# srv/pcl_feature_extraction

Hardware: AMD Instinct MI355X
Metric: Mpoints/s through NARF keypoint + FPFH descriptor on 1M-pt cloud (higher is better)
Workload: dtype f32; 1 GPU; configs[2] 1M-pt synthetic room, NARF(support 0.2) + normals(r 0.05) + FPFH(r 0.08) at the keypoints; image=640x480, parallelism=scan-per-gpu x1, descriptor_rows=83

## Files before the change

pcl_feature_extraction_amd/csrc/pfx_grid.hip:

```cpp
#include <algorithm>
#include <cstdlib>
#include <cstring>
#include <rocprim/rocprim.hpp>

#include "pfx_internal.h"

namespace pfx {
namespace {

__device__ __forceinline__ uint32_t f2ord(float f) {
  uint32_t u = __float_as_uint(f);
  return (u & 0x80000000u) ? ~u : (u | 0x80000000u);
}
__host__ __device__ __forceinline__ float ord2f(uint32_t u) {
  uint32_t b = (u & 0x80000000u) ? (u & 0x7fffffffu) : ~u;
  float f;
  memcpy(&f, &b, 4);
  return f;
}

constexpr int kBboxBlocks = 1024;
__global__ void __launch_bounds__(256) k_bbox(const float* __restrict__ x, const float* __restrict__ y,
                                              const float* __restrict__ z, int64_t n,
                                              uint32_t* __restrict__ mm) {
// ... 257 lines not shown

}

static bool bbox_dev(pfx_ctx* ctx, Grid& g, const float* d_x, const float* d_y, const float* d_z, int64_t n,
                     double lo[3], double hi[3]) {
  hipStream_t st = ctx->stream;
  uint32_t* mm = g.b_minmax.as<uint32_t>(6 * (kBboxBlocks + 1));
  const int blocks = (int)std::min<int64_t>(std::max<int64_t>(ceil_div(n, 1024), 1), kBboxBlocks);
  {
    TimeScope ts(ctx, "grid_bbox");
    k_bbox<<<blocks, 256, 0, st>>>(d_x, d_y, d_z, n, mm);
    k_bbox_reduce<<<1, 256, 0, st>>>(mm, blocks);
    check_launch("k_bbox");
  }
  uint32_t* h = ctx->readback<uint32_t>();
  PFX_HIP(hipMemcpyAsync(h, mm + 6 * blocks, sizeof(uint32_t) * 6, hipMemcpyDeviceToHost, st));
  ctx->sync_spin(st);
  uint32_t r[6];
  for (int d = 0; d < 6; ++d) r[d] = h[d];
  const bool any = r[0] != 0xffffffffu && r[3] != 0u;
  for (int d = 0; d < 3; ++d) {
    lo[d] = any ? ord2f(r[d]) : 0.0;
    hi[d] = any ? ord2f(r[3 + d]) : 0.0;
  }
  return any;
}

void points_bbox(pfx_ctx* ctx, Grid& g, const float* d_x, const float* d_y, const float* d_z, int64_t n,
                 double lo[3], double hi[3]) {
  bbox_dev(ctx, g, d_x, d_y, d_z, n, lo, hi);
}

void build_grid(pfx_ctx* ctx, Grid& g, const float* d_x, const float* d_y, const float* d_z,
                int64_t n, double radius, bool use_hint) {
  PFX_CHECK(n >= 0 && n < (int64_t(1) << 31), "point count must be in [0, 2^31)");
  PFX_CHECK(radius > 0.0, "radius must be > 0");
  if (&g == &ctx->grid_b) {
    ctx->prep_x = nullptr;
    ctx->prep_n = -1;
    ctx->prep_qx = nullptr;
    ctx->prep_nq = -1;
  }
  hipStream_t st = ctx->stream;
  ++g.gen;
  g.n = n;
  g.ux = d_x; g.uy = d_y; g.uz = d_z;
  double lo[3] = {0, 0, 0}, hi[3] = {0, 0, 0};
  g.oob = nullptr;
  g.hint_user |= use_hint;
  if (use_hint && g.have_hint && n > 0) {
    for (int d = 0; d < 3; ++d) {
      lo[d] = g.hint_lo[d];
      hi[d] = g.hint_hi[d];
    }
    g.oob = g.b_oob.as<int>(1);
  } else if (n > 0) {
    bbox_dev(ctx, g, d_x, d_y, d_z, n, lo, hi);
    for (int d = 0; d < 3; ++d) {
      const double m = 0.1 * (hi[d] - lo[d]) + 2.0 * radius;
      g.hint_lo[d] = lo[d] - m;
      g.hint_hi[d] = hi[d] + m;
    }
    g.have_hint = true;
  }
  double cell = radius * (1.0 + 1e-6);
  const double max_cells = double(1 << 26);
  int64_t dims[3];
  for (int it = 0; it < 64; ++it) {
    for (int d = 0; d < 3; ++d) dims[d] = (int64_t)std::floor((hi[d] - lo[d]) / cell) + 1;
// ... 50 lines not shown
    check_launch("k_count_keys");
    PFX_HIP(rocprim::exclusive_scan(tmp, scan_bytes, g.cell_start, g.cell_start, int32_t(0), (size_t)m,
                                    rocprim::plus<int32_t>(), st));
    k_count_scatter<<<(unsigned)blocks, kCountBlock, 0, st>>>(d_x, d_y, d_z, n, (uint32_t)C, keys, vals, g.cell_start,
                                                              scr, keys2);
    k_count_order<<<(unsigned)ceil_div(n, 256), 256, 0, st>>>(scr, keys2, n, (uint32_t)C, g.cell_start, g.perm, g.sx,
                                                              g.sy, g.sz, g.sp, g.oob);
    check_launch("k_count_order");
    return;
  }

  using SortCfg = rocprim::radix_sort_config<rocprim::default_config, rocprim::default_config,
                                             rocprim::default_config, 0>;
  int bits = 1;
  while ((int64_t(1) << bits) <= C) ++bits;
  size_t sort_bytes = 0, scan_bytes = 0;
  PFX_HIP(rocprim::radix_sort_pairs<SortCfg>(nullptr, sort_bytes, (uint32_t*)nullptr, (uint32_t*)nullptr,
                                    (uint32_t*)nullptr, (uint32_t*)nullptr, (size_t)std::max<int64_t>(n, 1),
                                    0, bits, st));
  auto rev = rocprim::make_reverse_iterator(static_cast<int32_t*>(nullptr));
  PFX_HIP(rocprim::inclusive_scan(nullptr, scan_bytes, rev, rev, (size_t)(C + 1), rocprim::minimum<int32_t>(), st));
  void* tmp = g.b_tmp.get(std::max(sort_bytes, scan_bytes) + 16);
  g.cell_start = g.b_start.as<int32_t>(C + 2);
  {
    TimeScope ts(ctx, "grid_build");
    k_fill_i32<<<(unsigned)std::min<int64_t>(ceil_div(C + 2, 256), 2048), 256, 0, st>>>(g.cell_start, C + 2,
                                                                                       (int32_t)n);
    if (g.oob) k_fill_i32<<<1, 64, 0, st>>>(g.oob, 1, 0);
    if (n > 0) {
      k_cell_keys<<<(unsigned)ceil_div(n, 256), 256, 0, st>>>(d_x, d_y, d_z, n, cm, keys, vals, g.oob);
      check_launch("k_cell_keys");
      PFX_HIP(rocprim::radix_sort_pairs<SortCfg>(tmp, sort_bytes, keys, keys2, vals,
                                        reinterpret_cast<uint32_t*>(g.perm), (size_t)n, 0, bits, st));
      k_mark_starts<<<(unsigned)ceil_div(n, 256), 256, 0, st>>>(keys2, n, g.cell_start);
      auto r = rocprim::make_reverse_iterator(g.cell_start + C + 1);
      PFX_HIP(rocprim::inclusive_scan(tmp, scan_bytes, r, r, (size_t)(C + 1), rocprim::minimum<int32_t>(), st));
      k_gather_sorted<<<(unsigned)ceil_div(n, 256), 256, 0, st>>>(
          d_x, d_y, d_z, n, reinterpret_cast<uint32_t*>(g.perm), g.sx, g.sy, g.sz, g.sp);
      check_launch("k_gather_sorted");
    }
  }
  if (!g.oob && n > 0 && g.hint_user) {
    int* d_fat = g.b_fat.as<int>(1);
    if (!g.h_fat) PFX_HIP(hipHostMalloc((void**)&g.h_fat, 64, hipHostMallocDefault));
    if (!g.fat_ev) PFX_HIP(hipEventCreateWithFlags(&g.fat_ev, hipEventDisableTiming));
    if (g.fat_pending) PFX_HIP(hipEventSynchronize(g.fat_ev));
    k_fill_i32<<<1, 64, 0, st>>>(d_fat, 1, 0);
    k_fat_cells<<<(unsigned)ceil_div(C, 256), 256, 0, st>>>(g.cell_start, C, d_fat);
    check_launch("k_fat_cells");
    PFX_HIP(hipMemcpyAsync(g.h_fat, d_fat, sizeof(int), hipMemcpyDeviceToHost, st));
    PFX_HIP(hipEventRecord(g.fat_ev, st));
    g.fat_pending = true;
  }
}

}
```

pcl_feature_extraction_amd/csrc/pfx_internal.h:

```cpp
#pragma once
#include <hip/hip_runtime.h>
#include <stdint.h>
#include <cstdlib>

#include <map>
#include <stdexcept>
#include <string>
#include <vector>

#include "../../include/pfx.h"

namespace pfx {

struct Error : std::runtime_error {
  pfx_status code;
  Error(pfx_status c, const std::string& m) : std::runtime_error(m), code(c) {}
};

#define PFX_HIP(expr)                                                                   \
  do {                                                                                  \
    hipError_t _e = (expr);                                                             \
    if (_e != hipSuccess)                                                               \
      throw ::pfx::Error(PFX_ERR_DEVICE, std::string(#expr) + ": " + hipGetErrorString(_e)); \
  } while (0)
// ... 129 lines not shown
  pfx::FpfhReadback* fpfh_rb() {
    if (!fpfh_rb_mem) PFX_HIP(hipHostMalloc(&fpfh_rb_mem, sizeof(pfx::FpfhReadback), hipHostMallocDefault));
    return static_cast<pfx::FpfhReadback*>(fpfh_rb_mem);
  }
  void* pfh_rb_mem = nullptr;
  bool pfh_pending = false;
  void* spin_rb_mem = nullptr;
  bool spin_pending = false;
  void* rift_rb_mem = nullptr;
  bool igrad_pending = false, rift_pending = false;
  void* sc_rb_mem = nullptr;
  bool sc_pending = false, lrf_pending = false;
  void* moments_rb_mem = nullptr;
  bool moments_pending = false, pcurv_pending = false;
  int64_t sc_rnd_n = 0;
  hipStream_t side = nullptr;
  hipEvent_t fork_ev[2] = {nullptr, nullptr};
  hipEvent_t spin_ev = nullptr;
  void sync_spin(hipStream_t st) {
    if (!spin_ev) PFX_HIP(hipEventCreateWithFlags(&spin_ev, hipEventDisableTiming));
    PFX_HIP(hipEventRecord(spin_ev, st));
    hipError_t e;
    while ((e = hipEventQuery(spin_ev)) == hipErrorNotReady) {
    }
    PFX_HIP(e);
  }
  void ensure_side() {
    if (side) return;
    int prio = 0;
    if (stream) PFX_HIP(hipStreamGetPriority(stream, &prio));
    PFX_HIP(hipStreamCreateWithPriority(&side, hipStreamNonBlocking, prio));
    for (auto& e : fork_ev) PFX_HIP(hipEventCreateWithFlags(&e, hipEventDisableTiming));
  }
  void* host_rb = nullptr;
  template <class T> T* readback() {
    if (!host_rb) PFX_HIP(hipHostMalloc(&host_rb, 4096, hipHostMallocDefault));
    return static_cast<T*>(host_rb);
  }
  void* host_scratch = nullptr;
  size_t host_scratch_bytes = 0;
  void* pinned(size_t need) {
    if (need > host_scratch_bytes) {
      if (host_scratch) {
        PFX_HIP(hipStreamSynchronize(stream));
        PFX_HIP(hipHostFree(host_scratch));
      }
      host_scratch_bytes = need + need / 2 + 4096;
      PFX_HIP(hipHostMalloc(&host_scratch, host_scratch_bytes, hipHostMallocDefault));
    }
    return host_scratch;
  }
};

namespace pfx {

struct TimeScope {
  pfx_ctx* ctx;
  hipEvent_t a = nullptr, b = nullptr;
  std::string name;
  TimeScope(pfx_ctx* c, std::string n, bool stage = false) : ctx(c), name(std::move(n)) {
    if (ctx->timer.enabled && (stage || !ctx->timer.stages_only)) {
      a = ctx->timer.take();
      b = ctx->timer.take();
      PFX_HIP(hipEventRecord(a, ctx->stream));
    }
  }
  ~TimeScope() {
    if (a) {
      (void)hipEventRecord(b, ctx->stream);
      ctx->timer.pending.push_back(KernelTimer::Pending{a, b, name});
    }
  }
};

inline void check_launch(const char* what) {
  hipError_t e = hipGetLastError();
  if (e != hipSuccess)
    throw Error(PFX_ERR_DEVICE, std::string("launch ") + what + ": " + hipGetErrorString(e));
}

inline int64_t ceil_div(int64_t a, int64_t b) { return (a + b - 1) / b; }

void build_grid(pfx_ctx* ctx, Grid& g, const float* d_x, const float* d_y, const float* d_z,
                int64_t n, double radius, bool use_hint = false);
void points_bbox(pfx_ctx* ctx, Grid& g, const float* d_x, const float* d_y, const float* d_z, int64_t n,
                 double lo[3], double hi[3]);
inline void note_grid_word(pfx_ctx* ctx, const Grid& g, int word) {
  if (!(word & kGridFatBit)) return;
  g.fat = true;
  ++ctx->stats["grid_fat_fallbacks"];
}
inline GridView view(const Grid& g) {
  GridView v;
  v.sx = g.sx; v.sy = g.sy; v.sz = g.sz; v.sp = g.sp; v.perm = g.perm; v.cell_start = g.cell_start;
  v.ux = g.ux; v.uy = g.uy; v.uz = g.uz;
  v.inv = g.dinv; v.ox = g.dox; v.oy = g.doy; v.oz = g.doz; v.nx = g.nx; v.ny = g.ny; v.nz = g.nz;
  return v;
}

void normals_dev(pfx_ctx* ctx, const float* x, const float* y, const float* z, int64_t n,
                 double r, const float vp[3], float* nx, float* ny, float* nz, float* curv);
void normals_lists_dev(pfx_ctx* ctx, const float* x, const float* y, const float* z, int64_t n, double r,
                       float* nx, float* ny, float* nz, float* curv);
void normals_chains_dev(pfx_ctx* ctx, pfx_ctx* owner, const uint8_t* mask, int want, const float vp[3], float* nx,
                        float* ny, float* nz, float* curv);
void normals_release(pfx_ctx* ctx);
void normals_grid_launch_dev(pfx_ctx* ctx, const float* x, const float* y, const float* z, int64_t n, double r);
void normals_launch_dev(pfx_ctx* ctx, const float* x, const float* y, const float* z, int64_t n, double r,
                        const float vp[3], float* nx, float* ny, float* nz, float* curv);
bool normals_finish_dev(pfx_ctx* ctx);
void normals_prepare_dev(pfx_ctx* ctx, const float* x, const float* y, const float* z, int64_t n, double r);
void normals_subset_dev(pfx_ctx* ctx, const float* x, const float* y, const float* z, int64_t n, double r,
                        const uint8_t* mask, int want, const float vp[3], float* nx, float* ny, float* nz,
                        float* curv);
void normals_fast_dev(pfx_ctx* ctx, const float* x, const float* y, const float* z, int64_t n, double r,
                      const float vp[3], float* nx, float* ny, float* nz, float* curv);
double cloud_resolution_dev(pfx_ctx* ctx, const float* x, const float* y, const float* z, int64_t n);
// ... 99 lines not shown
```

pcl_feature_extraction_amd/csrc/pfx_nblist.h:

```cpp
#pragma once
#include "pfx_internal.h"

namespace pfx {

constexpr uint32_t kEntryOffMask = 0x0fffffffu;
__host__ __device__ __forceinline__ int entry_run(uint32_t e) { return (int)(e >> 28); }
__host__ __device__ __forceinline__ uint32_t entry_off(uint32_t e) { return e & kEntryOffMask; }
constexpr uint8_t kLgCompact = 0x80;

__host__ __device__ __forceinline__ uint32_t widen_entry16(uint32_t e16) {
  return ((e16 >> 12) << 28) | (e16 & 0xfffu);
}
constexpr int kLaneMaxCompact = 2048;
__device__ __forceinline__ uint32_t list_entry(const uint32_t* list, int64_t off, int lgr, int m) {
  const int64_t i = off + ((int64_t)m << (lgr & 0x7f));
  return (lgr & kLgCompact) ? widen_entry16(reinterpret_cast<const uint16_t*>(list)[i]) : list[i];
}

struct NbLists {
  int64_t nq = 0;
  int64_t total = 0;
  int64_t long_total = 0;
  int64_t long_nq = 0;
  int64_t slots = 0;
  const int32_t* qpos = nullptr;
  const int64_t* off = nullptr;
  const int32_t* cnt = nullptr;
  const uint8_t* lg = nullptr;
  const uint32_t* list = nullptr;
  bool compact = false;
  int64_t list_cap = 0;
  const uint32_t* skeys = nullptr;
  const int64_t* nq_dev = nullptr;
};

__device__ __forceinline__ int64_t nq_of(const NbLists& L) { return L.nq_dev ? *L.nq_dev : L.nq; }

constexpr int kLongList = 1024;

struct NormalsState {
  NbLists L;
  int64_t n = 0;
  const float *x = nullptr, *y = nullptr, *z = nullptr;
  double r = 0.0;
  bool ready = false;
  uint64_t grid_gen = 0;
  bool pending = false;
  uint64_t grid_ahead_gen = 0;
  const float *grid_ahead_x = nullptr, *grid_ahead_y = nullptr, *grid_ahead_z = nullptr;
  int64_t grid_ahead_n = 0;
  double grid_ahead_r = 0.0;
  float vp[3] = {0.f, 0.f, 0.f};
  float *nx = nullptr, *ny = nullptr, *nz = nullptr, *curv = nullptr;
};

void build_lists(pfx_ctx* ctx, const Grid& g, const uint8_t* mask, double radius, bool sorted, NbLists& out,
                 const char* tag, bool defer = false, int want = 1, bool compact = false, bool gate = false);
bool build_lists_check(pfx_ctx* ctx, const Grid& g, NbLists& out, const char* tag);

}
```

pcl_feature_extraction_amd/csrc/pfx_nblist.hip:

```cpp
#include <cstdlib>
#include <cstring>
#include <rocprim/rocprim.hpp>

#include "pfx_nblist.h"
#include "pfx_neighbors.h"

namespace pfx {
namespace {

constexpr int kQ = 16;
typedef float pf2 __attribute__((ext_vector_type(2)));
constexpr int kArena = 16384;
constexpr int kArenaQuery = 16384;
constexpr int kTcapSmall = 384, kTcapSparse = 1280, kTcapDense = 8000;
constexpr int kCapQuery = 4096, kBucketsQuery = 1024;
constexpr int kCapMid8 = 8192, kBucketsMid8 = 1024;
constexpr int kCapMid = 16384, kBucketsMid = 2048;
#ifndef PFX_HUGE_BLOCKS
#define PFX_HUGE_BLOCKS 1024
#endif
constexpr int kCapHuge = 1 << 18, kBucketsHuge = 4096, kHugeBlocks = PFX_HUGE_BLOCKS;
#ifndef PFX_NT_QUERY
#define PFX_NT_QUERY 512
#endif
// ... 155 lines not shown
                                                    const int64_t* __restrict__ ntiles_ptr,
                                                    int32_t* __restrict__ recs, int64_t n,
                                                    int32_t* __restrict__ wide, int* __restrict__ counts) {
  const int64_t t = blockIdx.x * (int64_t)blockDim.x + threadIdx.x;
  const int64_t ntiles = *ntiles_ptr;
  const int lane = threadIdx.x & 63;
  int cls = -1, qn = 0;
  int32_t start = 0;
  Runs R;
  if (t < ntiles) {
    start = tiles[t];
    const int64_t next = (t + 1 < ntiles) ? tiles[t + 1] : *nq_ptr;
    qn = (int)(next - start < kQ ? next - start : kQ);
    const int T = block_runs(g, skeys[qpos[start]], R);
    cls = T <= kTcapSmall ? 3 : (T <= kTcapSparse ? 0 : (T <= kTcapDense ? 1 : 2));
  }
#pragma unroll
  for (int c = 0; c < 4; ++c) {
    const uint64_t m = __ballot(cls == c);
    if (!m) continue;
    int base = 0;
    const int ci = c == 3 ? kTilesSmall : (c == 2 ? kTilesWide : (c == 1 ? kTilesDense : kTilesSparse));
    if (lane == __builtin_ctzll(m)) base = atomicAdd(&counts[ci], __popcll(m));
    base = __shfl(base, __builtin_ctzll(m));
    if (cls == c) {
      const int64_t slot = base + __popcll(m & lanemask_lt());
      const int64_t at = c == 3 ? slot : (c == 0 ? n + slot : (c == 1 ? 2 * n - 1 - slot : n - 1 - slot));
      rec_write(recs + at * kRecInts, R, start, qn);
      if (c == 2) wide[slot] = (int32_t)at;
    }
  }
}

constexpr int kCoopTiles = 16;
constexpr int kCellsPerThread = 8;
constexpr int64_t kCellsMinGrid = int64_t(256) * 256 * kCellsPerThread;
__device__ __forceinline__ int tile_class(int T) {
  return T <= kTcapSmall ? 3 : (T <= kTcapSparse ? 0 : (T <= kTcapDense ? 1 : 2));
}
__global__ void __launch_bounds__(256) k_tile_cells(GridView g, int64_t ncells, int32_t* __restrict__ recs, int64_t n,
                                                    int32_t* __restrict__ wide, int* __restrict__ counts) {
  __shared__ int s_wave[4][4];
  __shared__ int s_base[4];
  const int lane = threadIdx.x & 63, wv = threadIdx.x >> 6;
  const int64_t c0 = (blockIdx.x * (int64_t)blockDim.x + threadIdx.x) * kCellsPerThread;
  int32_t st[kCellsPerThread + 1];
#pragma unroll
  for (int j = 0; j <= kCellsPerThread; ++j) st[j] = g.cell_start[c0 + j <= ncells ? c0 + j : ncells];
  int cnt[4] = {0, 0, 0, 0};
  unsigned cls_bits = 0;
#pragma unroll
  for (int j = 0; j < kCellsPerThread; ++j) {
    const int m = st[j + 1] - st[j];
    if (m > 0) {
      Runs R;
      const int cls = tile_class(block_runs(g, (uint32_t)(c0 + j), R));
      cls_bits |= (unsigned)cls << (2 * j);
#pragma unroll
      for (int k = 0; k < 4; ++k) cnt[k] += cls == k ? (m + kQ - 1) / kQ : 0;
    }
  }
  int first[4];
#pragma unroll
  for (int k = 0; k < 4; ++k) {
    const int incl = wave_incl_scan(cnt[k]);
    first[k] = incl - cnt[k];
    if (lane == 63) s_wave[k][wv] = incl;
  }
  __syncthreads();
  if (threadIdx.x < 4) {
    const int k = threadIdx.x;
    const int total = s_wave[k][0] + s_wave[k][1] + s_wave[k][2] + s_wave[k][3];
    const int ci = k == 3 ? kTilesSmall : (k == 2 ? kTilesWide : (k == 1 ? kTilesDense : kTilesSparse));
    s_base[k] = total ? atomicAdd(&counts[ci], total) : 0;
  }
  __syncthreads();
#pragma unroll
  for (int k = 0; k < 4; ++k) {
    first[k] += s_base[k];
    for (int w = 0; w < wv; ++w) first[k] += s_wave[k][w];
  }
  auto emit = [&](const Runs& Rc, int k, int slot, int32_t q0, int qn) {
    const int64_t at = k == 3 ? slot : (k == 0 ? n + slot : (k == 1 ? 2 * n - 1 - slot : n - 1 - slot));
    rec_write(recs + at * kRecInts, Rc, q0, qn);
    if (k == 2) wide[slot] = (int32_t)at;
  };
#pragma unroll
  for (int j = 0; j < kCellsPerThread; ++j) {
    const int32_t s = st[j], m = st[j + 1] - st[j];
    const int nt = (m + kQ - 1) / kQ, cls = (int)((cls_bits >> (2 * j)) & 3u);
    Runs R;
#pragma unroll
    for (int r = 0; r < 9; ++r) R.start[r] = 0;
#pragma unroll
    for (int r = 0; r < 10; ++r) R.pref[r] = 0;
    int slot = 0;
    if (m > 0) {
      block_runs(g, (uint32_t)(c0 + j), R);
      slot = cls == 3 ? first[3] : (cls == 2 ? first[2] : (cls == 1 ? first[1] : first[0]));
#pragma unroll
      for (int k = 0; k < 4; ++k) first[k] += cls == k ? nt : 0;
      if (nt <= kCoopTiles)
        for (int i = 0; i < nt; ++i) emit(R, cls, slot + i, s + kQ * i, min(kQ, m - kQ * i));
    }
    uint64_t big = __ballot(m > 0 && nt > kCoopTiles);
    while (big) {
      const int l = __builtin_ctzll(big);
      big &= big - 1;
      Runs Rl;
#pragma unroll
      for (int r = 0; r < 9; ++r) Rl.start[r] = __shfl(R.start[r], l);
#pragma unroll
      for (int r = 0; r < 10; ++r) Rl.pref[r] = __shfl(R.pref[r], l);
      const int32_t sl = __shfl(s, l), ml = __shfl(m, l);
      const int fl = __shfl(slot, l), ntl = __shfl(nt, l), kl = __shfl(cls, l);
      for (int i = lane; i < ntl; i += 64) emit(Rl, kl, fl + i, sl + kQ * i, min(kQ, ml - kQ * i));
    }
  }
}

struct ListOut {
  int64_t* off;
  int32_t* cnt;
  uint8_t* lg;
  uint32_t* list;
  unsigned long long* cursor;
  unsigned long long cap;
  int compact;
  int32_t* qrec;
};

struct CandLds {
  const float2* cxy;
  const float* cz;
  __device__ __forceinline__ void get(int t, float& x, float& y, float& z) const {
    const float2 v = cxy[t];
    x = v.x; y = v.y; z = cz[t];
  }
};
struct CandGlobal {
  const float4* sp;
  const Runs* R;
  __device__ __forceinline__ void get(int t, float& x, float& y, float& z) const {
    const float4 c = sp[run_pos(*R, t)];
    x = c.x; y = c.y; z = c.z;
  }
};

#ifdef PFX_SHOT_PROFILE
// ... 1238 lines not shown
    PFX_HIP(rocprim::select(nullptr, t3, rocprim::counting_iterator<int32_t>(0), flags, tiles, d_ntiles, (size_t)n,
                            st));
    tmp = buf("tmp").get(std::max(t1, std::max(t2, t3)) + 16);
    tq_dev = static_cast<TierQ*>(buf("tierq").get(sizeof(TierQ)));
    if (!lb.ptr) {
      size_t words = 64 * (size_t)(n + 1);
      if (const char* e = std::getenv("PFX_LIST_WORDS")) words = std::max<size_t>(256, std::strtoull(e, nullptr, 10));
      lb.get(sizeof(uint32_t) * words);
    }
    const int heavy = (int)std::min<int64_t>(4, n >> 21);
    ch_small = 4;
    ch_sparse = std::max(2, heavy);
    ch_dense = std::max(1, heavy);
  }

  size_t list_words() const { return lb.bytes / sizeof(uint32_t); }
  ListOut list_out() const {
    return ListOut{off, cnt, lgs, static_cast<uint32_t*>(lb.ptr), cursor, list_words(), compact, qrec};
  }

  void setup(const uint8_t* mask, int want) {
    const unsigned nb = (unsigned)ceil_div(n, 256);
    const TierQ tq{{q4k, q8k, q16k, qhuge},
                   {counters + kWork4k, counters + kWork8k, counters + kWork16k, counters + kWorkHuge}};
    TimeScope ts(ctx, std::string(tag) + "_tiles");
    if (mask) {
      k_list_init<<<1, 256, 0, st>>>(nullptr, 0, nullptr, d_nq, counters, kNCounters, cursor, tq, tq_dev);
      k_mask_flags<<<nb, 256, 0, st>>>(G.perm, G.skeys, n, (uint64_t)G.ncells, mask, want, flags);
      PFX_HIP(rocprim::select(tmp, t1, rocprim::counting_iterator<int32_t>(0), flags, qpos, d_nq, (size_t)n, st));
    } else {
      k_list_init<<<nb, 256, 0, st>>>(qpos, n, G.cell_start + G.ncells, d_nq, counters, kNCounters, cursor, tq,
                                      tq_dev);
      const char* mode = std::getenv("PFX_LIST_SETUP");
      const bool cells = mode && std::strcmp(mode, "cells") == 0
                             ? true
                             : (mode && std::strcmp(mode, "scan") == 0
                                    ? false
                                    : G.ncells >= kCellsMinGrid && G.ncells <= std::max<int64_t>(4 * n, kCellsMinGrid));
      ++ctx->stats[std::string(tag) + (cells ? "_setup_cells" : "_setup_scan")];
      if (cells) {
        k_tile_cells<<<(unsigned)ceil_div(G.ncells, 256 * kCellsPerThread), 256, 0, st>>>(g, G.ncells, recs, n, wq, counters);
        check_launch("nblist cell tiles");
        return;
      }
    }
    k_seg_marks<<<nb, 256, 0, st>>>(qpos, G.skeys, d_nq, seg);
    PFX_HIP(rocprim::inclusive_scan(tmp, t2, seg, seg, (size_t)n, rocprim::maximum<int32_t>(), st));
    k_tile_flags<<<nb, 256, 0, st>>>(seg, d_nq, flags, n);
    PFX_HIP(rocprim::select(tmp, t3, rocprim::counting_iterator<int32_t>(0), flags, tiles, d_ntiles, (size_t)n, st));
    k_tile_class<<<nb, 256, 0, st>>>(g, qpos, G.skeys, d_nq, tiles, d_ntiles, recs, n, wq, counters);
    check_launch("nblist tiles");
  }

  void reset_for_retry() {
    PFX_HIP(hipMemsetAsync(cursor, 0, 4 * sizeof(unsigned long long), st));
    PFX_HIP(hipMemsetAsync(counters + kRetryFirst, 0, (kNCounters - kRetryFirst) * sizeof(int), st));
  }

  template <int CAP, int NB, bool GLOBAL, int NT, int WPE>
  void launch_tier(unsigned grid, const int32_t* work, Counter count, Counter head, uint32_t* scratch,
                   const char* what) {
    const auto kern = k_nb_query<CAP, NB, GLOBAL, NT, WPE>;
    const size_t lds = GLOBAL ? 0 : sizeof(uint32_t) * 2 * CAP;
    if (lds) PFX_HIP(hipFuncSetAttribute((const void*)kern, hipFuncAttributeMaxDynamicSharedMemorySize, (int)lds));
    kern<<<grid, NT, lds, st>>>(g, work, counters + count, rr, (float)NB / rr, isort, list_out(),
                                GLOBAL ? nullptr : tq_dev, counters + kOverCap, scratch, counters + head);
    check_launch(what);
  }
  void launch_4k() {
    launch_tier<kCapQuery, kBucketsQuery, false, kNtQuery, PFX_Q_WPE>(kGrid4k, q4k, kWork4k, kHead4k, nullptr,
                                                                      "nblist 4k lists");
  }
  void launch_8k() {
    launch_tier<kCapMid8, kBucketsMid8, false, kNtMid8, kNtMid8 / 128>(kGrid8k, q8k, kWork8k, kHead8k, nullptr,
// ... 88 lines not shown
    out.lg = lgs;
    out.list = static_cast<const uint32_t*>(lb.ptr);
    out.compact = compact != 0;
    out.list_cap = (int64_t)list_words();
    out.skeys = G.skeys;
  }
};

}

bool build_lists_check(pfx_ctx* ctx, const Grid& G, NbLists& out, const char* tag) {
  auto B = [&](const char* what) -> DevBuf& { return ctx->bufs[bname(tag, what)]; };
  const ListsRb* rb = read_back(ctx, B("counters").ptr, B("cursor").ptr, B("nq").ptr, G.oob);
  note_grid_word(ctx, G, rb->oob);
  const size_t words = B("list").bytes / sizeof(uint32_t);
  const int ran = (int)ctx->stats[std::string(tag) + "_ran_mid_tiers"];
  const int lacking = lists_lack(rb->cnt, rb->cur[0], words, B("scratch").ptr != nullptr, ran, rb->oob);
  if (lacking & (kLackGrid | kLackBuffer | kLackScratch)) return false;
  note_mid_tiers(ctx, tag, rb->cnt);
  if (lacking) return false;
  if (rb->cnt[kOverCap] > 0) throw_over_cap(tag, rb->cnt[kOverCap]);
  publish(ctx, tag, *rb, words, out);
  return true;
}

void build_lists(pfx_ctx* ctx, const Grid& G, const uint8_t* mask, double radius, bool sorted, NbLists& out,
                 const char* tag, bool defer, int want, bool compact, bool gate) {
  out = NbLists();
  if (G.n == 0) return;
  if (G.n >= (int64_t(1) << 28))
    throw Error(PFX_ERR_CAPACITY, std::string(tag) + ": neighbour lists support < 2^28 points");
  ListBuild b(ctx, G, tag, radius, sorted, compact);
  b.setup(mask, want);
  if (gate && ctx->lists_gate) {
    PFX_HIP(hipStreamWaitEvent(b.st, ctx->lists_gate, 0));
    ctx->lists_gate = nullptr;
  }
  for (int attempt = 0; attempt < 3; ++attempt) {
    if (attempt) b.reset_for_retry();
    int ran = attempt ? kRanAll : wanted_tiers(ctx, tag);
    ctx->stats[std::string(tag) + "_ran_mid_tiers"] = ran;
    b.launch_lists(ran);
    if (defer && attempt == 0) {
      b.defer_to_check(ran, out);
      return;
    }
    const ListsRb* rb = b.read_back();
    int lacking = b.lack(rb, ran);
    if (lacking & kRanWide) {
      note_mid_tiers(ctx, tag, rb->cnt);
      ++ctx->stats[std::string(tag) + "_wide_reruns"];
      continue;
    }
    if (lacking & (kRan8k | kRan16k)) {
      b.catch_up(lacking, ran);
      ran = kRanAll;
      rb = b.read_back();
      lacking = b.lack(rb, ran);
      ++ctx->stats[std::string(tag) + "_tier_catchups"];
    }
    note_mid_tiers(ctx, tag, rb->cnt);
    const int n_huge = rb->cnt[kWorkHuge];
    if (lacking & kLackScratch) {
      b.huge_alloc(n_huge);
      b.launch_huge();
      rb = b.read_back();
// ... 22 lines not shown
```

pcl_feature_extraction_amd/csrc/pfx_normals.hip:

```cpp
#include <cstring>
#include <algorithm>
#include <cstdio>
#include <cstdlib>
#include <mutex>

#include <rocprim/rocprim.hpp>

#include "pfx_nblist.h"
#include "pfx_neighbors.h"
#include "pfx_normal_math.h"

namespace pfx {
namespace {

constexpr int kBatch = 8;
#ifndef PFX_LANE_MAX
#define PFX_LANE_MAX (2 * kLongList)
#endif
constexpr int kLaneMax = PFX_LANE_MAX;
static_assert(kLaneMax >= kLaneMaxCompact, "lists up to kLaneMaxCompact must take the lane-per-query chains");

#ifndef PFX_LANE_DENSE_MUL
#define PFX_LANE_DENSE_MUL 2
#endif
constexpr int kLaneMaxDense = PFX_LANE_DENSE_MUL * kLaneMax;

__device__ __forceinline__ void chain_add(float a[9], float x, float y, float z) {
  a[0] = a[0] + x * x;
  a[1] = a[1] + x * y;
  a[2] = a[2] + x * z;
  a[3] = a[3] + y * y;
  a[4] = a[4] + y * z;
  a[5] = a[5] + z * z;
  a[6] = a[6] + x;
  a[7] = a[7] + y;
  a[8] = a[8] + z;
}

__device__ __forceinline__ void store_normal(const GridView& g, int32_t p, const float a[9], int k, float vpx,
                                             float vpy, float vpz, float* nx, float* ny, float* nz, float* curv) {
  float o[4];
  const float4 q = g.sp[p];
  finish_normal(a, k, q.x, q.y, q.z, vpx, vpy, vpz, o);
  const int32_t orig = g.perm[p];
  nx[orig] = o[0];
  ny[orig] = o[1];
  nz[orig] = o[2];
  curv[orig] = o[3];
}

constexpr int kMaxCells = 64;
constexpr int kHash = 1024;
constexpr int kStageSmall = 3584;
constexpr int kStageBig = 12288;
constexpr int kMaxCols = kMaxCells * 9;
constexpr uint32_t kEmpty = 0xffffffffu;

template <int CAP>
// ... 346 lines not shown
                                                              int lane_max) {
  extern __shared__ __attribute__((aligned(16))) unsigned char dyn[];
  ChainLds<kStageBig>& S = *reinterpret_cast<ChainLds<kStageBig>*>(dyn);
  const int count = modes[3];
  for (int w = blockIdx.x; w < count; w += gridDim.x) {
    __syncthreads();
    chain_wg<kStageBig, false>(S, g, L, deferq[w], vpx, vpy, vpz, nx, ny, nz, curv, longq, n_long, modes, nullptr,
                               mask, want, lane_max);
  }
}

#ifndef PFX_LONG_LB
#define PFX_LONG_LB 64
#endif
constexpr int kPerWave = 7, kLB = PFX_LONG_LB, kLR = kLB / 32;
static_assert(kLB % 32 == 0, "whole 32-step halves");
constexpr int kLongWgPerCu = kLB <= 32 ? 4 : 3;
#ifndef PFX_BIG_GRID
#define PFX_BIG_GRID 256
#endif
#ifndef PFX_LONG_ORDERED
#define PFX_LONG_ORDERED 1
#endif
#ifndef PFX_LONG_GRID_MUL
#define PFX_LONG_GRID_MUL 1
#endif
constexpr int kLBPad = kLB + 4;
struct LongLds {
  float c[2][3][kPerWave][kLBPad];
  int32_t rtab[kPerWave * 9];
};

__global__ void k_nan_fill4(float* __restrict__ a, float* __restrict__ b, float* __restrict__ c,
                            float* __restrict__ d, int64_t n) {
  const float v = __builtin_nanf("");
  for (int64_t i = blockIdx.x * (int64_t)blockDim.x + threadIdx.x; i < n; i += (int64_t)gridDim.x * blockDim.x) {
    a[i] = v; b[i] = v; c[i] = v; d[i] = v;
  }
}

__global__ void k_nan_fill4_masked(float* __restrict__ a, float* __restrict__ b, float* __restrict__ c,
                                   float* __restrict__ d, int64_t n, const uint8_t* __restrict__ mask, int want) {
  const float v = __builtin_nanf("");
  for (int64_t i = blockIdx.x * (int64_t)blockDim.x + threadIdx.x; i < n; i += (int64_t)gridDim.x * blockDim.x) {
    if ((mask[i] != 0) != (want != 0)) continue;
    a[i] = v; b[i] = v; c[i] = v; d[i] = v;
  }
}

__global__ void __launch_bounds__(256) k_long_lists(GridView g, NbLists L, const uint8_t* __restrict__ mask, int want,
                                                    int lane_max,
                                                    int32_t* __restrict__ longq, int* __restrict__ n_long,
                                                    uint8_t* __restrict__ flags) {
  const int64_t j = blockIdx.x * (int64_t)blockDim.x + threadIdx.x;
  bool push = false;
  if (want >= 2 && mask) {
    const bool sel = j < nq_of(L) && mask[g.perm[L.qpos[j]]] != 0;
    const bool mine = (__syncthreads_or(sel) != 0) == ((want & 1) != 0);
    push = mine && j < nq_of(L) && L.cnt[j] > lane_max;
  } else if (j < nq_of(L) && L.cnt[j] > lane_max) {
    push = !mask || ((mask[g.perm[L.qpos[j]]] != 0) == (want != 0));
  }
  if (flags) {
    flags[j] = push ? 1 : 0;
  } else if (push) {
    longq[wave_push_slot(n_long)] = (int32_t)j;
  }
}
// ... 131 lines not shown
  }
}

}



struct GateScope {
  pfx_ctx* ctx;
  explicit GateScope(pfx_ctx* c) : ctx(c) {}
  ~GateScope() { ctx->lists_gate = nullptr; }
};

void normals_release(pfx_ctx* ctx) {
  delete ctx->normals;
  ctx->normals = nullptr;
}

void normals_lists_dev(pfx_ctx* ctx, const float* x, const float* y, const float* z, int64_t n, double r,
                       float* nx, float* ny, float* nz, float* curv) {
  GateScope gate_scope(ctx);
  PFX_CHECK(r > 0.0, "normals: radius must be > 0");
  PFX_CHECK(n >= 0, "normals: negative point count");
  if (!ctx->normals) ctx->normals = new NormalsState();
  NormalsState& ns = *ctx->normals;
  ns.ready = false;
  ns.pending = false;
  ns.n = n;
  ns.x = x;
  ns.y = y;
  ns.z = z;
  ns.r = r;
  ns.L = NbLists();
  if (n == 0) {
    ns.ready = true;
    return;
  }
  hipStream_t st = ctx->stream;
  TimeScope total(ctx, "normals_lists_phase", true);
  build_grid(ctx, ctx->grid_a, x, y, z, n, r);
  k_nan_fill4<<<(unsigned)std::min<int64_t>(ceil_div(n, 256), 4096), 256, 0, st>>>(nx, ny, nz, curv, n);
  check_launch("k_nan_fill4");
  build_lists(ctx, ctx->grid_a, nullptr, r, true, ns.L, "normals", false, 1, false, true);
  ctx->stats["normals_neighbors"] = ns.L.total;
  ctx->stats["normals_long_neighbors"] = ns.L.long_total;
  ctx->stats["normals_long_queries"] = ns.L.long_nq;
  ctx->stats["normals_queries"] = ns.L.nq;
  ns.ready = true;
}

void normals_chains_dev(pfx_ctx* ctx, pfx_ctx* owner, const uint8_t* mask, int want, const float vp[3], float* nx,
                        float* ny, float* nz, float* curv) {
  PFX_CHECK(owner->normals && owner->normals->ready, "normals: lists not built (call the lists phase first)");
  const NbLists& L = owner->normals->L;
  if (L.nq == 0) return;
  hipStream_t st = ctx->stream;
  const Grid& G = owner->grid_a;
  int32_t* longq = ctx->buf("normals_longq").as<int32_t>(L.nq);
  int* n_long = ctx->buf("normals_nlong").as<int>(5);
  PFX_HIP(hipMemsetAsync(n_long, 0, 5 * sizeof(int), st));
  const int64_t nb = ceil_div(L.nq, 256);
  const bool fork = L.nq_dev ? ctx->normals_fork_hint : L.long_nq * 8 <= L.nq;
  if (!L.nq_dev) ctx->normals_fork_hint = fork;
  const int lane_max = fork ? kLaneMax : kLaneMaxDense;
  if (fork || !PFX_LONG_ORDERED) {
    k_long_lists<<<(unsigned)nb, 256, 0, st>>>(view(G), L, mask, want, lane_max, longq, n_long, nullptr);
    check_launch("k_long_lists");
  } else {
    uint8_t* flags = ctx->buf("normals_longflag").as<uint8_t>(nb * 256);
    k_long_lists<<<(unsigned)nb, 256, 0, st>>>(view(G), L, mask, want, lane_max, longq, n_long, flags);
    check_launch("k_long_lists");
    size_t tb = 0;
    PFX_HIP(rocprim::select(nullptr, tb, rocprim::counting_iterator<int32_t>(0), flags, longq, n_long,
                            (size_t)L.nq, st));
    void* tmp = ctx->buf("normals_longsel").get(tb + 16);
    PFX_HIP(rocprim::select(tmp, tb, rocprim::counting_iterator<int32_t>(0), flags, longq, n_long, (size_t)L.nq,
                            st));
  }
  const int64_t lb = std::min<int64_t>(ceil_div(L.nq, 7 * 4), 256 * kLongWgPerCu * PFX_LONG_GRID_MUL);
  if (fork) {
    ctx->ensure_side();
    PFX_HIP(hipEventRecord(ctx->fork_ev[0], st));
    PFX_HIP(hipStreamWaitEvent(ctx->side, ctx->fork_ev[0], 0));
    k_normals_long<<<(unsigned)lb, 256, 0, ctx->side>>>(view(G), L, longq, n_long, vp[0], vp[1], vp[2], nx, ny, nz,
                                                        curv);
    check_launch("k_normals_long");
  }
  {
    int64_t* deferq = ctx->buf("normals_deferq").as<int64_t>(nb);
    {
      TimeScope ts(ctx, "normals_chain");
      k_normals_chain<<<(unsigned)nb, 256, 0, st>>>(view(G), L, vp[0], vp[1], vp[2], nx, ny, nz, curv, longq, n_long,
                                                    n_long + 1, deferq, mask, want, lane_max);
// ... 37 lines not shown
    unsigned long long pr[16];
    PFX_HIP(hipStreamSynchronize(st));
    PFX_HIP(hipMemcpyFromSymbol(pr, HIP_SYMBOL(g_chain_prof), sizeof(pr)));
    for (int b = 0; b < 16; b += 8)
      fprintf(stderr, "chain%s: WGs %llu prologue %.0f cyc/WG | waves %llu chain %.0f cyc/wave, max k %.1f/wave, "
              "%.1f cyc/step, mean k %.1f/lane\n", b ? "_big" : "", pr[b + 4], pr[b + 0] / (double)(pr[b + 4] + !pr[b + 4]), pr[b + 3],
              pr[b + 1] / (double)(pr[b + 3] + !pr[b + 3]), pr[b + 2] / (double)(pr[b + 3] + !pr[b + 3]),
              pr[b + 1] / (double)(pr[b + 2] + !pr[b + 2]), pr[b + 5] / 64.0 / (double)(pr[b + 3] + !pr[b + 3]));
    const unsigned long long z[16] = {};
    PFX_HIP(hipMemcpyToSymbol(HIP_SYMBOL(g_chain_prof), z, sizeof(z)));
  }
#endif
}

namespace {

bool normals_speculative_lists(pfx_ctx* ctx, const float* x, const float* y, const float* z, int64_t n, double r,
                               float* nx, float* ny, float* nz, float* curv) {
  if (n == 0) return false;
  if (!ctx->normals) ctx->normals = new NormalsState();
  NormalsState& ns = *ctx->normals;
  ns.ready = false;
  ns.pending = false;
  ns.n = n;
  ns.x = x;
  ns.y = y;
  ns.z = z;
  ns.r = r;
  ns.L = NbLists();
  TimeScope phase(ctx, "normals_lists_phase", true);
  const bool ahead = ns.grid_ahead_gen != 0 && ns.grid_ahead_gen == ctx->grid_a.gen && ns.grid_ahead_x == x &&
                     ns.grid_ahead_y == y && ns.grid_ahead_z == z && ns.grid_ahead_n == n && ns.grid_ahead_r == r;
  ns.grid_ahead_gen = 0;
  if (!ahead) build_grid(ctx, ctx->grid_a, x, y, z, n, r, true);
  k_nan_fill4<<<(unsigned)std::min<int64_t>(ceil_div(n, 256), 4096), 256, 0, ctx->stream>>>(nx, ny, nz, curv, n);
  check_launch("k_nan_fill4");
  build_lists(ctx, ctx->grid_a, nullptr, r, true, ns.L, "normals", true, 1, true,
              true);
  return true;
}

bool normals_conclude(pfx_ctx* ctx, bool ok, const float* x, const float* y, const float* z, int64_t n, double r,
                      const float vp[3], float* nx, float* ny, float* nz, float* curv) {
  NormalsState& ns = *ctx->normals;
  ctx->grid_a.oob = nullptr;
  ctx->stats["normals_speculative_reruns"] += ok ? 0 : 1;
  if (ok) {
    ctx->stats["normals_neighbors"] = ns.L.total;
    ctx->stats["normals_long_neighbors"] = ns.L.long_total;
    ctx->stats["normals_long_queries"] = ns.L.long_nq;
    ctx->stats["normals_queries"] = ns.L.nq;
    ctx->normals_fork_hint = ns.L.long_nq * 8 <= ns.L.nq;
    return true;
  }
  normals_lists_dev(ctx, x, y, z, n, r, nx, ny, nz, curv);
  normals_chains_dev(ctx, ctx, nullptr, 0, vp, nx, ny, nz, curv);
  return false;
}
}

void normals_dev(pfx_ctx* ctx, const float* x, const float* y, const float* z, int64_t n, double r,
                 const float vp[3], float* nx, float* ny, float* nz, float* curv) {
  GateScope gate_scope(ctx);
  TimeScope total(ctx, "normals", true);
  PFX_CHECK(r > 0.0, "normals: radius must be > 0");
  PFX_CHECK(n >= 0, "normals: negative point count");
  if (normals_speculative_lists(ctx, x, y, z, n, r, nx, ny, nz, curv)) {
    NormalsState& ns = *ctx->normals;
    const bool ok = build_lists_check(ctx, ctx->grid_a, ns.L, "normals");
// ... 105 lines not shown
```

Before: 216.0 Mpoints/s.

## Fork sorted gather to side stream and rebuild cell tiling from sorted keys

During the speculative normals grid build, the sorted-coordinate gather and the NaN fill now run on a side stream, overlapping with mark-starts, the scan and list setup. A join before list construction and at scope exit restores ordering. The NaN fill also zeroes the long-query counters, so the separate memset is dropped. The cell-tiling kernel is rewritten to walk sorted point keys in slices with shared-memory staging and coalesced record writes, and it is now the default setup path instead of a heuristic choice. The risk is race bugs if the side-stream joins are missed, plus added shared-memory pressure in the tiling kernel.

```diff
diff --git a/pcl_feature_extraction_amd/csrc/pfx_grid.hip b/pcl_feature_extraction_amd/csrc/pfx_grid.hip
--- a/pcl_feature_extraction_amd/csrc/pfx_grid.hip
+++ b/pcl_feature_extraction_amd/csrc/pfx_grid.hip
@@ -313,9 +313,10 @@
 }
 
 void build_grid(pfx_ctx* ctx, Grid& g, const float* d_x, const float* d_y, const float* d_z,
-                int64_t n, double radius, bool use_hint) {
+                int64_t n, double radius, bool use_hint, bool fork_gather) {
   PFX_CHECK(n >= 0 && n < (int64_t(1) << 31), "point count must be in [0, 2^31)");
   PFX_CHECK(radius > 0.0, "radius must be > 0");
+  ctx->join_side(ctx->stream);
   if (&g == &ctx->grid_b) {
     ctx->prep_x = nullptr;
     ctx->prep_n = -1;
@@ -432,12 +433,18 @@
       check_launch("k_cell_keys");
       PFX_HIP(rocprim::radix_sort_pairs<SortCfg>(tmp, sort_bytes, keys, keys2, vals,
                                         reinterpret_cast<uint32_t*>(g.perm), (size_t)n, 0, bits, st));
+      const bool forked = fork_gather && g.oob != nullptr;
+      if (forked) ctx->fork_side(st);
+      const auto gather = [&](hipStream_t s) {
+        k_gather_sorted<<<(unsigned)ceil_div(n, 256), 256, 0, s>>>(d_x, d_y, d_z, n, reinterpret_cast<uint32_t*>(g.perm),
+                                                                   g.sx, g.sy, g.sz, g.sp);
+        check_launch("k_gather_sorted");
+      };
+      if (forked) gather(ctx->side);
       k_mark_starts<<<(unsigned)ceil_div(n, 256), 256, 0, st>>>(keys2, n, g.cell_start);
       auto r = rocprim::make_reverse_iterator(g.cell_start + C + 1);
       PFX_HIP(rocprim::inclusive_scan(tmp, scan_bytes, r, r, (size_t)(C + 1), rocprim::minimum<int32_t>(), st));
-      k_gather_sorted<<<(unsigned)ceil_div(n, 256), 256, 0, st>>>(
-          d_x, d_y, d_z, n, reinterpret_cast<uint32_t*>(g.perm), g.sx, g.sy, g.sz, g.sp);
-      check_launch("k_gather_sorted");
+      if (!forked) gather(st);
     }
   }
   if (!g.oob && n > 0 && g.hint_user) {
diff --git a/pcl_feature_extraction_amd/csrc/pfx_internal.h b/pcl_feature_extraction_amd/csrc/pfx_internal.h
--- a/pcl_feature_extraction_amd/csrc/pfx_internal.h
+++ b/pcl_feature_extraction_amd/csrc/pfx_internal.h
@@ -185,6 +185,19 @@
     PFX_HIP(hipStreamCreateWithPriority(&side, hipStreamNonBlocking, prio));
     for (auto& e : fork_ev) PFX_HIP(hipEventCreateWithFlags(&e, hipEventDisableTiming));
   }
+  bool side_pending = false;
+  void fork_side(hipStream_t st) {
+    ensure_side();
+    PFX_HIP(hipEventRecord(fork_ev[0], st));
+    PFX_HIP(hipStreamWaitEvent(side, fork_ev[0], 0));
+    side_pending = true;
+  }
+  void join_side(hipStream_t st) {
+    if (!side_pending) return;
+    side_pending = false;
+    PFX_HIP(hipEventRecord(fork_ev[1], side));
+    PFX_HIP(hipStreamWaitEvent(st, fork_ev[1], 0));
+  }
   void* host_rb = nullptr;
   template <class T> T* readback() {
     if (!host_rb) PFX_HIP(hipHostMalloc(&host_rb, 4096, hipHostMallocDefault));
@@ -235,7 +248,7 @@
 inline int64_t ceil_div(int64_t a, int64_t b) { return (a + b - 1) / b; }
 
 void build_grid(pfx_ctx* ctx, Grid& g, const float* d_x, const float* d_y, const float* d_z,
-                int64_t n, double radius, bool use_hint = false);
+                int64_t n, double radius, bool use_hint = false, bool fork_gather = false);
 void points_bbox(pfx_ctx* ctx, Grid& g, const float* d_x, const float* d_y, const float* d_z, int64_t n,
                  double lo[3], double hi[3]);
 inline void note_grid_word(pfx_ctx* ctx, const Grid& g, int word) {
diff --git a/pcl_feature_extraction_amd/csrc/pfx_nblist.h b/pcl_feature_extraction_amd/csrc/pfx_nblist.h
--- a/pcl_feature_extraction_amd/csrc/pfx_nblist.h
+++ b/pcl_feature_extraction_amd/csrc/pfx_nblist.h
@@ -46,6 +46,7 @@
   bool ready = false;
   uint64_t grid_gen = 0;
   bool pending = false;
+  bool nlong_zeroed = false;
   uint64_t grid_ahead_gen = 0;
   const float *grid_ahead_x = nullptr, *grid_ahead_y = nullptr, *grid_ahead_z = nullptr;
   int64_t grid_ahead_n = 0;
diff --git a/pcl_feature_extraction_amd/csrc/pfx_nblist.hip b/pcl_feature_extraction_amd/csrc/pfx_nblist.hip
--- a/pcl_feature_extraction_amd/csrc/pfx_nblist.hip
+++ b/pcl_feature_extraction_amd/csrc/pfx_nblist.hip
@@ -211,89 +211,142 @@
   }
 }
 
-constexpr int kCoopTiles = 16;
-constexpr int kCellsPerThread = 8;
-constexpr int64_t kCellsMinGrid = int64_t(256) * 256 * kCellsPerThread;
+constexpr int kSlicePerThread = 16;
+constexpr int kSlice = 256 * kSlicePerThread;
+constexpr int kRunCells = 128;
 __device__ __forceinline__ int tile_class(int T) {
   return T <= kTcapSmall ? 3 : (T <= kTcapSparse ? 0 : (T <= kTcapDense ? 1 : 2));
 }
-__global__ void __launch_bounds__(256) k_tile_cells(GridView g, int64_t ncells, int32_t* __restrict__ recs, int64_t n,
-                                                    int32_t* __restrict__ wide, int* __restrict__ counts) {
-  __shared__ int s_wave[4][4];
+__device__ __forceinline__ void runs_store(int32_t* __restrict__ o, const Runs& R) {
+#pragma unroll
+  for (int r = 0; r < 9; ++r) o[r] = R.start[r];
+#pragma unroll
+  for (int r = 0; r < 10; ++r) o[9 + r] = R.pref[r];
+}
+__global__ void __launch_bounds__(256) k_tile_cells(GridView g, const uint32_t* __restrict__ skeys, int64_t ncells,
+                                                    int32_t* __restrict__ recs, int64_t n, int32_t* __restrict__ wide,
+                                                    int* __restrict__ counts) {
+  __shared__ int32_t s_pos[kSlice + 1];
+  __shared__ int32_t s_tile[kSlice + 1];
+  __shared__ int32_t s_slot[kSlice];
+  __shared__ int32_t s_runs[kRunCells][kRecQ0];
+  __shared__ int32_t s_tat[256], s_tcell[256], s_tq0[256], s_tqn[256];
+  __shared__ int s_wave[5][4];
   __shared__ int s_base[4];
-  const int lane = threadIdx.x & 63, wv = threadIdx.x >> 6;
-  const int64_t c0 = (blockIdx.x * (int64_t)blockDim.x + threadIdx.x) * kCellsPerThread;
-  int32_t st[kCellsPerThread + 1];
-#pragma unroll
-  for (int j = 0; j <= kCellsPerThread; ++j) st[j] = g.cell_start[c0 + j <= ncells ? c0 + j : ncells];
-  int cnt[4] = {0, 0, 0, 0};
-  unsigned cls_bits = 0;
-#pragma unroll
-  for (int j = 0; j < kCellsPerThread; ++j) {
-    const int m = st[j + 1] - st[j];
-    if (m > 0) {
+  const int tid = threadIdx.x, lane = tid & 63, wv = tid >> 6;
+  const int64_t i0 = blockIdx.x * (int64_t)kSlice + (int64_t)tid * kSlicePerThread;
+  uint32_t key[kSlicePerThread];
+  if (i0 + kSlicePerThread <= n) {
+    const uint4* k4 = reinterpret_cast<const uint4*>(skeys + i0);
+#pragma unroll
+    for (int j = 0; j < kSlicePerThread / 4; ++j) {
+      const uint4 v = k4[j];
+      key[4 * j] = v.x; key[4 * j + 1] = v.y; key[4 * j + 2] = v.z; key[4 * j + 3] = v.w;
+    }
+  } else {
+#pragma unroll
+    for (int j = 0; j < kSlicePerThread; ++j) key[j] = i0 + j < n ? skeys[i0 + j] : 0xffffffffu;
+  }
+  uint32_t prev = (i0 > 0 && i0 < n) ? skeys[i0 - 1] : 0xffffffffu;
+  unsigned starts = 0;
+#pragma unroll
+  for (int j = 0; j < kSlicePerThread; ++j) {
+    starts |= ((uint64_t)key[j] < (uint64_t)ncells && key[j] != prev) ? 1u << j : 0u;
+    prev = key[j];
+  }
+  {
+    const int mine = __popc(starts), incl = wave_incl_scan(mine);
+    if (lane == 63) s_wave[4][wv] = incl;
+    __syncthreads();
+    int at = incl - mine;
+    for (int w = 0; w < wv; ++w) at += s_wave[4][w];
+#pragma unroll
+    for (int j = 0; j < kSlicePerThread; ++j)
+      if (starts >> j & 1u) s_pos[at++] = (int32_t)(i0 + j);
+  }
+  const int cells = s_wave[4][0] + s_wave[4][1] + s_wave[4][2] + s_wave[4][3];
+  __syncthreads();
+  if (cells == 0) return;
+  int before[5] = {0, 0, 0, 0, 0};
+  for (int c0 = 0; c0 < cells; c0 += 256) {
+    const int c = c0 + tid;
+    int nt = 0, cls = 0;
+    if (c < cells) {
+      const int32_t pos = s_pos[c];
+      const uint32_t k = skeys[pos];
+      const int32_t end = g.cell_start[(int64_t)k + 1];
+      if (c == cells - 1) s_pos[cells] = end;
+      nt = (end - pos + kQ - 1) / kQ;
       Runs R;
-      const int cls = tile_class(block_runs(g, (uint32_t)(c0 + j), R));
-      cls_bits |= (unsigned)cls << (2 * j);
-#pragma unroll
-      for (int k = 0; k < 4; ++k) cnt[k] += cls == k ? (m + kQ - 1) / kQ : 0;
-    }
-  }
-  int first[4];
-#pragma unroll
-  for (int k = 0; k < 4; ++k) {
-    const int incl = wave_incl_scan(cnt[k]);
-    first[k] = incl - cnt[k];
-    if (lane == 63) s_wave[k][wv] = incl;
+      cls = tile_class(block_runs(g, k, R));
+      if (c < kRunCells) runs_store(s_runs[c], R);
+    }
+    int ex[5];
+#pragma unroll
+    for (int k = 0; k < 5; ++k) {
+      const int v = (k == 4 || cls == k) ? nt : 0, incl = wave_incl_scan(v);
+      ex[k] = incl - v;
+      if (lane == 63) s_wave[k][wv] = incl;
+    }
+    __syncthreads();
+#pragma unroll
+    for (int k = 0; k < 5; ++k) {
+      ex[k] += before[k];
+      for (int w = 0; w < 4; ++w) {
+        ex[k] += w < wv ? s_wave[k][w] : 0;
+        before[k] += s_wave[k][w];
+      }
+    }
+    if (c < cells) {
+      s_tile[c] = ex[4];
+      s_slot[c] = (int32_t)((uint32_t)cls << 30) | (cls == 3 ? ex[3] : (cls == 2 ? ex[2] : (cls == 1 ? ex[1] : ex[0])));
+    }
+    __syncthreads();
+  }
+  if (tid == 0) s_tile[cells] = before[4];
+  if (tid < 4) {
+    const int ci = tid == 3 ? kTilesSmall : (tid == 2 ? kTilesWide : (tid == 1 ? kTilesDense : kTilesSparse));
+    const int total = tid == 3 ? before[3] : (tid == 2 ? before[2] : (tid == 1 ? before[1] : before[0]));
+    s_base[tid] = total ? atomicAdd(&counts[ci], total) : 0;
   }
   __syncthreads();
-  if (threadIdx.x < 4) {
-    const int k = threadIdx.x;
-    const int total = s_wave[k][0] + s_wave[k][1] + s_wave[k][2] + s_wave[k][3];
-    const int ci = k == 3 ? kTilesSmall : (k == 2 ? kTilesWide : (k == 1 ? kTilesDense : kTilesSparse));
-    s_base[k] = total ? atomicAdd(&counts[ci], total) : 0;
-  }
-  __syncthreads();
-#pragma unroll
-  for (int k = 0; k < 4; ++k) {
-    first[k] += s_base[k];
-    for (int w = 0; w < wv; ++w) first[k] += s_wave[k][w];
-  }
-  auto emit = [&](const Runs& Rc, int k, int slot, int32_t q0, int qn) {
-    const int64_t at = k == 3 ? slot : (k == 0 ? n + slot : (k == 1 ? 2 * n - 1 - slot : n - 1 - slot));
-    rec_write(recs + at * kRecInts, Rc, q0, qn);
-    if (k == 2) wide[slot] = (int32_t)at;
-  };
-#pragma unroll
-  for (int j = 0; j < kCellsPerThread; ++j) {
-    const int32_t s = st[j], m = st[j + 1] - st[j];
-    const int nt = (m + kQ - 1) / kQ, cls = (int)((cls_bits >> (2 * j)) & 3u);
-    Runs R;
-#pragma unroll
-    for (int r = 0; r < 9; ++r) R.start[r] = 0;
-#pragma unroll
-    for (int r = 0; r < 10; ++r) R.pref[r] = 0;
-    int slot = 0;
-    if (m > 0) {
-      block_runs(g, (uint32_t)(c0 + j), R);
-      slot = cls == 3 ? first[3] : (cls == 2 ? first[2] : (cls == 1 ? first[1] : first[0]));
-#pragma unroll
-      for (int k = 0; k < 4; ++k) first[k] += cls == k ? nt : 0;
-      if (nt <= kCoopTiles)
-        for (int i = 0; i < nt; ++i) emit(R, cls, slot + i, s + kQ * i, min(kQ, m - kQ * i));
-    }
-    uint64_t big = __ballot(m > 0 && nt > kCoopTiles);
-    while (big) {
-      const int l = __builtin_ctzll(big);
-      big &= big - 1;
-      Runs Rl;
-#pragma unroll
-      for (int r = 0; r < 9; ++r) Rl.start[r] = __shfl(R.start[r], l);
-#pragma unroll
-      for (int r = 0; r < 10; ++r) Rl.pref[r] = __shfl(R.pref[r], l);
-      const int32_t sl = __shfl(s, l), ml = __shfl(m, l);
-      const int fl = __shfl(slot, l), ntl = __shfl(nt, l), kl = __shfl(cls, l);
-      for (int i = lane; i < ntl; i += 64) emit(Rl, kl, fl + i, sl + kQ * i, min(kQ, ml - kQ * i));
+  for (int c0 = 0; c0 < cells; c0 += kRunCells) {
+    const int c1 = min(cells, c0 + kRunCells);
+    if (c0 > 0 && tid < c1 - c0) {
+      Runs R;
+      block_runs(g, skeys[s_pos[c0 + tid]], R);
+      runs_store(s_runs[tid], R);
+    }
+    __syncthreads();
+    const int t1 = s_tile[c1];
+    for (int tb = s_tile[c0]; tb < t1; tb += 256) {
+      const int nt = min(256, t1 - tb);
+      if (tid < nt) {
+        const int t = tb + tid;
+        int lo = c0, hi = c1 - 1;
+        while (lo < hi) {
+          const int mid = (lo + hi + 1) >> 1;
+          if (s_tile[mid] <= t) lo = mid; else hi = mid - 1;
+        }
+        const int ti = t - s_tile[lo], k = (int)((uint32_t)s_slot[lo] >> 30);
+        const int slot = s_base[k] + (s_slot[lo] & 0x3fffffff) + ti;
+        const int32_t pos = s_pos[lo], m = s_pos[lo + 1] - pos;
+        const int64_t at = k == 3 ? slot : (k == 0 ? n + slot : (k == 1 ? 2 * n - 1 - slot : n - 1 - slot));
+        s_tat[tid] = (int32_t)at;
+        s_tcell[tid] = lo - c0;
+        s_tq0[tid] = pos + kQ * ti;
+        s_tqn[tid] = min(kQ, m - kQ * ti);
+        if (k == 2) wide[slot] = (int32_t)at;
+      }
+      __syncthreads();
+      const int words = nt * kRecInts;
+#pragma unroll 4
+      for (int idx = tid; idx < words; idx += 256) {
+        const int tl = idx / kRecInts, w = idx - tl * kRecInts;
+        const int32_t v = w < kRecQ0 ? s_runs[s_tcell[tl]][w] : (w == kRecQ0 ? s_tq0[tl] : (w == kRecQn ? s_tqn[tl] : 0));
+        recs[(int64_t)s_tat[tl] * kRecInts + w] = v;
+      }
+      __syncthreads();
     }
   }
 }
@@ -1598,14 +1651,10 @@
       k_list_init<<<nb, 256, 0, st>>>(qpos, n, G.cell_start + G.ncells, d_nq, counters, kNCounters, cursor, tq,
                                       tq_dev);
       const char* mode = std::getenv("PFX_LIST_SETUP");
-      const bool cells = mode && std::strcmp(mode, "cells") == 0
-                             ? true
-                             : (mode && std::strcmp(mode, "scan") == 0
-                                    ? false
-                                    : G.ncells >= kCellsMinGrid && G.ncells <= std::max<int64_t>(4 * n, kCellsMinGrid));
+      const bool cells = !(mode && std::strcmp(mode, "scan") == 0);
       ++ctx->stats[std::string(tag) + (cells ? "_setup_cells" : "_setup_scan")];
       if (cells) {
-        k_tile_cells<<<(unsigned)ceil_div(G.ncells, 256 * kCellsPerThread), 256, 0, st>>>(g, G.ncells, recs, n, wq, counters);
+        k_tile_cells<<<(unsigned)ceil_div(n, kSlice), 256, 0, st>>>(g, G.skeys, G.ncells, recs, n, wq, counters);
         check_launch("nblist cell tiles");
         return;
       }
@@ -1760,6 +1809,7 @@
     throw Error(PFX_ERR_CAPACITY, std::string(tag) + ": neighbour lists support < 2^28 points");
   ListBuild b(ctx, G, tag, radius, sorted, compact);
   b.setup(mask, want);
+  ctx->join_side(b.st);
   if (gate && ctx->lists_gate) {
     PFX_HIP(hipStreamWaitEvent(b.st, ctx->lists_gate, 0));
     ctx->lists_gate = nullptr;
diff --git a/pcl_feature_extraction_amd/csrc/pfx_normals.hip b/pcl_feature_extraction_amd/csrc/pfx_normals.hip
--- a/pcl_feature_extraction_amd/csrc/pfx_normals.hip
+++ b/pcl_feature_extraction_amd/csrc/pfx_normals.hip
@@ -24,6 +24,7 @@
 #define PFX_LANE_DENSE_MUL 2
 #endif
 constexpr int kLaneMaxDense = PFX_LANE_DENSE_MUL * kLaneMax;
+constexpr int kNLong = 5;
 
 __device__ __forceinline__ void chain_add(float a[9], float x, float y, float z) {
   a[0] = a[0] + x * x;
@@ -436,8 +437,9 @@
 };
 
 __global__ void k_nan_fill4(float* __restrict__ a, float* __restrict__ b, float* __restrict__ c,
-                            float* __restrict__ d, int64_t n) {
+                            float* __restrict__ d, int64_t n, int* __restrict__ zero, int nzero) {
   const float v = __builtin_nanf("");
+  if (blockIdx.x == 0 && (int)threadIdx.x < nzero) zero[threadIdx.x] = 0;
   for (int64_t i = blockIdx.x * (int64_t)blockDim.x + threadIdx.x; i < n; i += (int64_t)gridDim.x * blockDim.x) {
     a[i] = v; b[i] = v; c[i] = v; d[i] = v;
   }
@@ -635,6 +637,7 @@
   ns.z = z;
   ns.r = r;
   ns.L = NbLists();
+  ns.nlong_zeroed = false;
   if (n == 0) {
     ns.ready = true;
     return;
@@ -642,7 +645,7 @@
   hipStream_t st = ctx->stream;
   TimeScope total(ctx, "normals_lists_phase", true);
   build_grid(ctx, ctx->grid_a, x, y, z, n, r);
-  k_nan_fill4<<<(unsigned)std::min<int64_t>(ceil_div(n, 256), 4096), 256, 0, st>>>(nx, ny, nz, curv, n);
+  k_nan_fill4<<<(unsigned)std::min<int64_t>(ceil_div(n, 256), 4096), 256, 0, st>>>(nx, ny, nz, curv, n, nullptr, 0);
   check_launch("k_nan_fill4");
   build_lists(ctx, ctx->grid_a, nullptr, r, true, ns.L, "normals", false, 1, false, true);
   ctx->stats["normals_neighbors"] = ns.L.total;
@@ -660,8 +663,10 @@
   hipStream_t st = ctx->stream;
   const Grid& G = owner->grid_a;
   int32_t* longq = ctx->buf("normals_longq").as<int32_t>(L.nq);
-  int* n_long = ctx->buf("normals_nlong").as<int>(5);
-  PFX_HIP(hipMemsetAsync(n_long, 0, 5 * sizeof(int), st));
+  int* n_long = ctx->buf("normals_nlong").as<int>(kNLong);
+  NormalsState& own = *owner->normals;
+  if (!(ctx == owner && own.nlong_zeroed)) PFX_HIP(hipMemsetAsync(n_long, 0, kNLong * sizeof(int), st));
+  own.nlong_zeroed = false;
   const int64_t nb = ceil_div(L.nq, 256);
   const bool fork = L.nq_dev ? ctx->normals_fork_hint : L.long_nq * 8 <= L.nq;
   if (!L.nq_dev) ctx->normals_fork_hint = fork;
@@ -765,9 +770,24 @@
   const bool ahead = ns.grid_ahead_gen != 0 && ns.grid_ahead_gen == ctx->grid_a.gen && ns.grid_ahead_x == x &&
                      ns.grid_ahead_y == y && ns.grid_ahead_z == z && ns.grid_ahead_n == n && ns.grid_ahead_r == r;
   ns.grid_ahead_gen = 0;
-  if (!ahead) build_grid(ctx, ctx->grid_a, x, y, z, n, r, true);
-  k_nan_fill4<<<(unsigned)std::min<int64_t>(ceil_div(n, 256), 4096), 256, 0, ctx->stream>>>(nx, ny, nz, curv, n);
+  struct SideJoin {
+    pfx_ctx* ctx;
+    ~SideJoin() {
+      try {
+        ctx->join_side(ctx->stream);
+      } catch (...) {
+      }
+    }
+  } side_join{ctx};
+  const char* fork_env = std::getenv("PFX_GATHER_FORK");
+  const bool fork_gather = !(fork_env && std::strcmp(fork_env, "0") == 0);
+  if (!ahead) build_grid(ctx, ctx->grid_a, x, y, z, n, r, true, fork_gather);
+  ctx->stats["normals_gather_forked"] += ctx->side_pending ? 1 : 0;
+  int* n_long = ctx->buf("normals_nlong").as<int>(kNLong);
+  k_nan_fill4<<<(unsigned)std::min<int64_t>(ceil_div(n, 256), 4096), 256, 0,
+                ctx->side_pending ? ctx->side : ctx->stream>>>(nx, ny, nz, curv, n, n_long, kNLong);
   check_launch("k_nan_fill4");
+  ns.nlong_zeroed = true;
   build_lists(ctx, ctx->grid_a, nullptr, r, true, ns.L, "normals", true, 1, true,
               true);
   return true;
```

New measurement: 220.2 Mpoints/s (median of 6 runs). +2.0%, better.
